# david-cortes/poismf

Measured on AMD Instinct MI355X. Metric: nonzeros/sec per full A+B sweep, higher is better.
Workload: dtype f32; 1 GPU; uniform 1000000x100000, 99949803 nnz (100000000 triplets, seed 1, duplicates summed), k=50, method=pg, maxupd=10, l2=1000, step=1e-09

## Files before the change

poismf_amd/csrc/poismf_hip.hip:

```cpp
#include <hip/hip_runtime.h>

#include <algorithm>
#include <atomic>
#include <cstdio>
#include <cstdlib>
#include <type_traits>

#include "plan.hpp"
#include "reg_eval.hpp"
#include "quad_eval.hpp"
#include "lane_eval.hpp"
#include "solvers.hpp"

#ifndef PMF_TU
#define PMF_TU -1
#endif
constexpr bool tu_has(int kmethod) { return PMF_TU == -1 || PMF_TU == kmethod; }

template <class EV, class = void> struct cold_constants : std::false_type {};
template <class EV> struct cold_constants<EV, std::void_t<decltype(EV::COLD_CONSTANTS)>> : std::integral_constant<bool, EV::COLD_CONSTANTS> {};

template <class EV, class = void> struct has_idle_tile : std::false_type {};
template <class EV> struct has_idle_tile<EV, std::void_t<decltype(&EV::idle_tile)>> : std::true_type {};

template <class EV, class T, int NC, int METHOD>
__device__ __forceinline__ void solve_row(const HalfArgs<T>& a, EV& ev, const T (&bs)[NC], unsigned lrow, unsigned nnz)
{
    const int k = a.geom.k;
    T* out = a.M + (size_t)(a.row_offset + lrow) * (size_t)k;
    T* out_p = a.Mp != nullptr ? a.Mp + (size_t)(a.row_offset + lrow) * (size_t)a.ldM : nullptr;
    T x[NC];
    if (nnz == 0) {
        T z = (T)0;
        asm volatile("" : "+v"(z));
        PMF_EW x[i] = z;
        ev.store_vec(out, x);
        if (out_p != nullptr) ev.store_vec(out_p, x);
        return;
    }
    ev.start_point(out, x);
    ev.n_eval = 0;

    T shift[NC];
    PMF_EW shift[i] = bs[i];
    const bool weighted = a.P.w != (T)1;
    if (weighted) {
        T cs[NC];
        PMF_EW cs[i] = (T)0;
        ev.tile_colsum(cs);
        T w_here = a.P.w;
        asm volatile("" : "+v"(w_here));
        const T wm1 = w_here - (T)1.;
        PMF_EW {
            shift[i] = cs[i] * wm1;
            shift[i] = shift[i] + bs[i];
        }
        if (METHOD == K_PG) {
            PMF_EW shift[i] = shift[i] * a.P.neg_step;
            if (a.P.neg_step2 != (T)1) { PMF_EW shift[i] = shift[i] * a.P.neg_step2; }
        }
    }

    SolveStats st;
    if constexpr (METHOD == K_EVAL) {
        T g[NC];
        double f;
        if (a.P.maxupd == 0) {
            f = (double)fun_single(ev, a.P, shift, x);
            grad_single(ev, a.P, shift, x, g, weighted);
        } else f = (double)fun_and_grad(ev, a.P, shift, x, g);
        ev.store_vec(out, g);
        if (out_p != nullptr) ev.store_vec(out_p, g);
        if (a.dec_rows != nullptr && ev.lane == 0 && ev.wid == 0 && ev.member == 0) {
            const unsigned long long fb = __builtin_bit_cast(unsigned long long, f);
            a.dec_rows[2 * (size_t)lrow] = (unsigned)fb;
            a.dec_rows[2 * (size_t)lrow + 1] = (unsigned)(fb >> 32);
        }
        return;
    } else if constexpr (METHOD == K_PG) {
        pg_row(ev, a.P, x, shift);
    } else if constexpr (METHOD == K_CG) {
        if constexpr (EV::MAY_CACHE) {
            if (a.P.limit_step && ev.pq_cap > 0 && nnz <= (unsigned)ev.pq_cap) cg_row_cached(ev, a.P, shift, x, weighted, st);
            else cg_row(ev, a.P, shift, x, weighted, st);
        } else cg_row(ev, a.P, shift, x, weighted, st);
    } else {
        T prev[NC];
        PMF_EW prev[i] = x[i];
        if (!a.reuse_prev) { PMF_EW x[i] = (T)1e-3; }
        (void)Tnc<T, NC, EV>::minimize(ev, a.P, shift, x, st);
        if (a.early_stop) {
            PMF_EW prev[i] = prev[i] - x[i];
            const T moved = ev.dot(prev, prev);
            if ((double)moved <= 1e-4 && ev.lane == 0 && ev.wid == 0 && ev.member == 0) atomicAdd(a.n_unchanged, 1u);
        }
    }
    ev.store_vec(out, x);
    if (out_p != nullptr) ev.store_vec(out_p, x);
#ifndef PMF_PROBE
    if (a.eval_rows != nullptr && ev.lane == 0 && ev.wid == 0 && ev.member == 0) a.eval_rows[lrow] += ev.n_eval;
#endif
    if (a.dec_rows != nullptr && ev.lane == 0 && ev.wid == 0 && ev.member == 0) {
        unsigned d0 = (unsigned)st.niter | ((unsigned)st.rc << 24), d1 = (unsigned)st.nfeval;
        if constexpr (cold_constants<EV>::value) asm volatile("" : "+v"(d0), "+v"(d1));
        a.dec_rows[2 * (size_t)lrow] = d0;
        a.dec_rows[2 * (size_t)lrow + 1] = d1;
    }
}

template <int METHOD, class T> __device__ __forceinline__ unsigned take_ticket(const HalfArgs<T>& a)
{
    unsigned st = 0u;
    if constexpr (METHOD != K_PG) {
        if (a.stop != nullptr) st = __hip_atomic_load(a.stop, __ATOMIC_RELAXED, __HIP_MEMORY_SCOPE_SYSTEM);
    }
    const unsigned t = atomicAdd(a.queue, 1u);
    return st != 0u ? 0xffffffffu : t;
}

template <class EV, class T, int NC, int METHOD, int NW>
__device__ __forceinline__ void sweep_rows(const HalfArgs<T>& a, EV& ev, unsigned char* smem)
{
    if (a.gate != nullptr && __hip_atomic_load(a.gate, __ATOMIC_RELAXED, __HIP_MEMORY_SCOPE_AGENT) == 0) return;
    ev.init(a.geom, a.F, smem);
    T bs[NC];
    ev.load_vec(a.bsum, bs);
    const RowDesc* desc = a.desc + a.perm_begin;
    if constexpr (EV::PIPELINED && (EV::PIPE_MW == 1 || (EV::PIPE_MW == 2 && METHOD == K_PG))) {
        unsigned r = blockIdx.x;
        auto ticket = [&]() -> unsigned {
            if (a.queue != nullptr) {
                if constexpr (NW > 1) {
                    unsigned* slot = ev.ticket_slot();
                    if (threadIdx.x == 0) *slot = take_ticket<METHOD>(a);
                    __syncthreads();
                    const unsigned t = uniform(*slot);
                    __syncthreads();
                    return t;
                }
                unsigned t = 0;
                if (ev.lane == 0) t = take_ticket<METHOD>(a);
                return uniform(t);
            }
            unsigned t = r;
            r += gridDim.x;
            if constexpr (METHOD != K_PG) {
                if (a.stop != nullptr && __hip_atomic_load(a.stop, __ATOMIC_RELAXED, __HIP_MEMORY_SCOPE_SYSTEM) != 0u) t = 0xffffffffu;
            }
            return t;
        };
        auto fetch = [&](unsigned t) -> RowDesc { return desc[t < a.nrows ? t : 0u]; };
        unsigned t0 = ticket(), t1 = ticket();
        RowDesc d0 = fetch(t0), d1 = fetch(t1);
        if (t0 < a.nrows) ev.fetch_meta(a.indices + (((unsigned long long)d0.p0_hi << 32) | d0.p0_lo), d0.nnz);
#ifdef PMF_PROBE
        unsigned probe_i = 0;
#endif
        while (t0 < a.nrows) {
            const unsigned long long p0 = ((unsigned long long)d0.p0_hi << 32) | d0.p0_lo;
            if (d0.nnz != 0) ev.gather(a.values + p0, d0.nnz);
            else if constexpr (has_idle_tile<EV>::value) ev.idle_tile();
            const unsigned t2 = ticket();
            const RowDesc d2 = fetch(t2);
            if (t1 < a.nrows) ev.fetch_meta(a.indices + (((unsigned long long)d1.p0_hi << 32) | d1.p0_lo), d1.nnz);
#ifdef PMF_PROBE
            ev.probe = (a.eval_rows != nullptr && blockIdx.x == 5 && threadIdx.x < WAVE && probe_i < 60) ? a.eval_rows + 16 * probe_i : nullptr;
            if (ev.probe != nullptr && ev.lane == 0) { ev.probe[10] = (unsigned)__builtin_amdgcn_s_memtime(); ev.probe[11] = d0.nnz; }
            probe_i++;
#endif
            solve_row<EV, T, NC, METHOD>(a, ev, bs, d0.lrow, d0.nnz);
            t0 = t1; d0 = d1;
            t1 = t2; d1 = d2;
        }
        return;
    } else {
        unsigned r = blockIdx.x;
        for (;;) {
            if (a.queue != nullptr) {
                if constexpr (NW > 1) {
                    unsigned* next_row = ev.ticket_slot();
                    if (threadIdx.x == 0) *next_row = take_ticket<METHOD>(a);
                    __syncthreads();
                    r = uniform(*next_row);
                    __syncthreads();
                } else {
                    unsigned t = 0;
                    if (ev.lane == 0) t = take_ticket<METHOD>(a);
                    r = uniform(t);
                }
            }
            if (r >= a.nrows) break;
            if constexpr (METHOD != K_PG) {
                if (a.queue == nullptr && a.stop != nullptr && uniform(__hip_atomic_load(a.stop, __ATOMIC_RELAXED, __HIP_MEMORY_SCOPE_SYSTEM)) != 0u) break;
            }
            const RowDesc d = desc[r];
            r += gridDim.x;
            const unsigned nnz = uniform(d.nnz);
            const unsigned long long p0 = ((unsigned long long)uniform(d.p0_hi) << 32) | uniform(d.p0_lo);
            if (nnz != 0) ev.begin_row(a.indices + p0, a.values + p0, nnz);
            solve_row<EV, T, NC, METHOD>(a, ev, bs, uniform(d.lrow), nnz);
        }
    }
}

template <class T, int NC, int METHOD, int SL, int NW>
__global__ __launch_bounds__(WAVE* NW) void half_sweep_kernel(const HalfArgs<T> a)
{
    extern __shared__ __attribute__((aligned(16))) unsigned char smem[];
    constexpr bool PF = SL > 0 && METHOD != K_TNCG;
    RowEval<T, NC, SL, NW, PF> ev;
    if constexpr (NW > 1) {
        if (a.arrive != nullptr && threadIdx.x == 0) atomicAdd(a.arrive, 1u);
    }
#ifdef PMF_TIMING
    const unsigned long long t_kernel = __builtin_amdgcn_s_memtime();
#endif
    sweep_rows<RowEval<T, NC, SL, NW, PF>, T, NC, METHOD, NW>(a, ev, smem);
#ifdef PMF_TIMING
    ev.tacc[5] = __builtin_amdgcn_s_memtime() - t_kernel;
    if (ev.lane == 0 && ev.wid == 0)
        for (int q = 0; q < 6; q++) atomicAdd(&g_pmf_timing[q], ev.tacc[q]);
#endif
}

template <class EV, class T, int NC, int METHOD>
__device__ __forceinline__ void team_rows(const HalfArgs<T>& a, EV& ev, unsigned char* smem)
{
    if (a.arrive != nullptr && threadIdx.x == 0) atomicAdd(a.arrive, 1u);
    ev.init(a.geom, a.F, smem);
    T bs[NC];
    ev.load_vec(a.bsum, bs);
    const RowDesc* desc = a.desc + a.perm_begin;
    const unsigned M = a.team_members;
    unsigned* box = ev.ticket_slot();
    if (threadIdx.x == 0) {
        const unsigned n = atomicAdd((unsigned*)a.team_buf, 1u);
        box[0] = n / M;
        box[1] = n % M;
    }
    __syncthreads();
    const unsigned team = uniform(box[0]);
    ev.member = (int)uniform(box[1]);
    __syncthreads();
    if ((size_t)(team + 1) * gt_team_words(M) + GT_HEAD_WORDS > GT_BUF_BYTES / 8) return;
    ev.tm_M = (int)M;
    ev.tm_seq = 0;
    ev.tm_words = a.team_buf + GT_HEAD_WORDS + (size_t)team * gt_team_words(M);
    ev.tm_err = a.team_err;
    ev.tm_spin = a.team_spin;
    unsigned long long* mail = ev.tm_words;
    constexpr unsigned END = 0xffffffffu;
    if (threadIdx.x == 0) atomicAdd((unsigned*)(mail + 2), 1u);
    if (a.team_spin <= 1u && threadIdx.x == 0) __hip_atomic_store(a.team_err, 1u, __ATOMIC_RELAXED, __HIP_MEMORY_SCOPE_AGENT);
    if (ev.wid == 0) {
        for (unsigned spins = 0;; spins++) {
            if (a.team_spin <= 1u) break;
            if (uniform((unsigned)gt_load(mail + 2)) >= M) break;
            if ((spins & 255u) == 255u) {
                if (uniform(__hip_atomic_load(a.team_err, __ATOMIC_RELAXED, __HIP_MEMORY_SCOPE_AGENT)) != 0) break;
                if (uniform(__hip_atomic_load(a.queue, __ATOMIC_RELAXED, __HIP_MEMORY_SCOPE_AGENT)) >= a.nrows) break;
            }
            if ((spins >> 6) > a.team_spin) { __hip_atomic_store(a.team_err, 1u, __ATOMIC_RELAXED, __HIP_MEMORY_SCOPE_AGENT); break; }
            __builtin_amdgcn_s_sleep(8);
        }
    }
    __syncthreads();
    for (unsigned rowno = 1;; rowno++) {
        if (ev.wid == 0) {
            unsigned tk = END;
            if (ev.member == 0) {
                unsigned t0 = 0;
                if (ev.lane == 0) t0 = take_ticket<METHOD>(a);
                tk = uniform(t0);
                if (tk >= a.nrows || uniform(__hip_atomic_load(a.team_err, __ATOMIC_RELAXED, __HIP_MEMORY_SCOPE_AGENT)) != 0) tk = END;
                gt_store(mail + (rowno & 1u), ((unsigned long long)rowno << 32) | tk);
            } else {
                unsigned seen = uniform(__hip_atomic_load(a.queue, __ATOMIC_RELAXED, __HIP_MEMORY_SCOPE_AGENT));
                for (unsigned spins = 0;; spins++) {
                    const unsigned long long v = gt_load(mail + (rowno & 1u));
                    const unsigned hi = uniform((unsigned)(v >> 32)), lo = uniform((unsigned)v);
                    if (hi == rowno) { tk = lo; break; }
                    if ((spins & 255u) == 255u) {
                        if (uniform(__hip_atomic_load(a.team_err, __ATOMIC_RELAXED, __HIP_MEMORY_SCOPE_AGENT)) != 0) break;
                        const unsigned q = uniform(__hip_atomic_load(a.queue, __ATOMIC_RELAXED, __HIP_MEMORY_SCOPE_AGENT));
                        if (q != seen) { seen = q; spins = 0; }
                        else if (rowno == 1u && q >= a.nrows) break;
                    }
                    if (spins > a.team_spin) { __hip_atomic_store(a.team_err, 1u, __ATOMIC_RELAXED, __HIP_MEMORY_SCOPE_AGENT); break; }
                    __builtin_amdgcn_s_sleep(4);
                }
            }
            box[0] = tk;
        }
        __syncthreads();
        const unsigned t = uniform(box[0]);
        __syncthreads();
        if (t >= a.nrows) break;
        const RowDesc d = desc[t];
        const unsigned nnz = uniform(d.nnz);
        const unsigned long long p0 = ((unsigned long long)uniform(d.p0_hi) << 32) | uniform(d.p0_lo);
        const unsigned S = ((nnz + M - 1u) / M + (EV::TEAM_ROUND - 1u)) / EV::TEAM_ROUND * EV::TEAM_ROUND;
        const unsigned off = (unsigned)ev.member * S;
        const unsigned mine = off < nnz ? (nnz - off < S ? nnz - off : S) : 0u;
        ev.begin_row(a.indices + p0 + (mine ? off : 0u), a.values + p0 + (mine ? off : 0u), mine);
        solve_row<EV, T, NC, METHOD>(a, ev, bs, uniform(d.lrow), nnz);
    }
}
template <class T, int NC, int METHOD, int SL, int NW>
__global__ __launch_bounds__(WAVE* NW) void half_sweep_giant_kernel(const HalfArgs<T> a)
{
    extern __shared__ __attribute__((aligned(16))) unsigned char smem[];
    constexpr bool PF = SL > 0 && METHOD != K_TNCG;
    using EV = RowEval<T, NC, SL, NW, PF, true>;
    EV ev;
    team_rows<EV, T, NC, METHOD>(a, ev, smem);
}
template <class T, int METHOD, int KS, int LV, int LA, int LL, int NW, int LP>
__global__ __launch_bounds__(WAVE* NW) __attribute__((amdgpu_waves_per_eu(1, 1))) void half_sweep_lane_team_kernel(const HalfArgs<T> a)
{
    using EV = LaneEval<T, KS, LV, LA, LL, NW, false, LP, 0, true>;
    __shared__ __attribute__((aligned(16))) unsigned char smem[EV::SMEM_BYTES];
    EV ev;
    team_rows<EV, T, EV::NC, METHOD>(a, ev, smem);
}

#ifndef PMF_PG_EXTRA
#define PMF_PG_EXTRA 56
#endif
#ifndef PMF_CG_EXTRA
#define PMF_CG_EXTRA 120
#endif
#ifndef PMF_TNC_EXTRA
#define PMF_TNC_EXTRA 100
#endif
constexpr int reg_waves(int tile_regs, int method)
{
    const int need = tile_regs + (method == K_PG ? PMF_PG_EXTRA : method == K_CG ? PMF_CG_EXTRA : PMF_TNC_EXTRA);
    for (int w : { 8, 6, 5, 4, 3, 2 })
        if ((512 / w) / 8 * 8 >= need) return w;
    return 1;
}
template <class T, int METHOD, int G, int NS> constexpr bool reg_pairs() { return METHOD == K_PG && sizeof(T) == 4 && G == 16 && NS == 1; }
template <class T, int METHOD, int S, int G, int NS>
__global__ __launch_bounds__(WAVE) __attribute__((amdgpu_waves_per_eu(reg_waves(4 * S * NS, METHOD)))) void half_sweep_reg_kernel(const HalfArgs<T> a)
{
    using EV = RegEval<T, S, G, NS, 1, 1, reg_pairs<T, METHOD, G, NS>()>;
    EV ev;
    constexpr int SMEM = EV::SMEM_BYTES;
    __shared__ __attribute__((aligned(16))) unsigned char smem[SMEM > 0 && METHOD == K_CG ? SMEM : 16];
#ifdef PMF_TIMING
    const unsigned long long t_kernel = __builtin_amdgcn_s_memtime();
#endif
    sweep_rows<EV, T, EV::NC, METHOD, 1>(a, ev, smem);
#ifdef PMF_TIMING
    if (ev.lane == 0) atomicAdd(&g_pmf_timing[5], __builtin_amdgcn_s_memtime() - t_kernel);
#endif
}

template <int Q>
__global__ __launch_bounds__(WAVE) __attribute__((amdgpu_waves_per_eu(reg_waves(14 * Q, K_PG)))) void half_sweep_quad_kernel(const HalfArgs<float> a)
{
    using EV = QuadEval<Q>;
    EV ev;
    sweep_rows<EV, float, EV::NC, K_PG, 1>(a, ev, nullptr);
}

constexpr int regw_waves(int tile_regs, int method, int nw)
{
    const int w = reg_waves(tile_regs + (method == K_PG ? 8 : 0), method);
    return nw >= 16 && w < 4 ? 4 : (nw >= 8 && w < 2 ? 2 : w);
}
template <class T, int METHOD, int S, int G, int NS, int NW>
__global__ __launch_bounds__(WAVE* NW) __attribute__((amdgpu_waves_per_eu(regw_waves(4 * S * NS, METHOD, NW)))) void half_sweep_regw_kernel(const HalfArgs<T> a)
{
    using EV = RegEval<T, S, G, NS, NW>;
    __shared__ __attribute__((aligned(16))) unsigned char smem[EV::SMEM_BYTES];
    EV ev;
    sweep_rows<EV, T, EV::NC, METHOD, NW>(a, ev, smem);
}

template <class T, int METHOD, int S, int G, int NS, int NW, int M>
__global__ __launch_bounds__(WAVE* NW) __attribute__((amdgpu_waves_per_eu(1))) void half_sweep_team_kernel(const HalfArgs<T> a)
{
    using EV = RegEval<T, S, G, NS, NW, M>;
    constexpr int NC = EV::NC;
    __shared__ __attribute__((aligned(16))) unsigned char smem[EV::SMEM_BYTES];
    EV ev;
    ev.init(a.geom, a.F, smem);
    T bs[NC];
    ev.load_vec(a.bsum, bs);
    const RowDesc* desc = a.desc + a.perm_begin;
    unsigned* arrive = (unsigned*)a.team_buf;
    unsigned* err = a.team_err;
    unsigned* box = ev.ticket_slot();
    if (threadIdx.x == 0) {
        unsigned xcc = 0;
        if (gridDim.x >= 8u * 4u * (unsigned)M) {
            asm volatile("s_getreg_b32 %0, hwreg(HW_REG_XCC_ID)" : "=s"(xcc));
            xcc &= 7u;
        }
        const unsigned n = atomicAdd(arrive + xcc, 1u);
        box[0] = xcc * TEAM_SLOTS_PER_XCD + n / (unsigned)M;
        box[1] = n % (unsigned)M;
        if (n / (unsigned)M >= TEAM_SLOTS_PER_XCD) __hip_atomic_store(err, 2u, __ATOMIC_RELAXED, __HIP_MEMORY_SCOPE_AGENT);
    }
    __syncthreads();
    const unsigned team = uniform(box[0]) % TEAM_SLOTS;
    ev.member = (int)uniform(box[1]);
    __syncthreads();
    ev.team_words = a.team_buf + TEAM_HEAD_WORDS + (size_t)team * TEAM_WORDS;
    ev.team_err = err;
    ev.team_spin = a.team_spin;
    unsigned long long* mail = ev.team_words;
    unsigned long long* here = ev.team_words + 2;
    constexpr unsigned END = 0xffffffffu;
    if (ev.member != 0 && threadIdx.x == 0) gran_store(here + ev.member, 1ull);

    if (ev.member == 0) {
        if (threadIdx.x == 0) {
            unsigned full = 0;
            unsigned seen = __hip_atomic_load(a.queue, __ATOMIC_RELAXED, __HIP_MEMORY_SCOPE_AGENT);
            for (unsigned spins = 0; !full; spins++) {
                full = 1;
                for (int m = 1; m < M; m++) full &= gran_load(here + m) != 0ull;
                if (full) break;
                const unsigned q = __hip_atomic_load(a.queue, __ATOMIC_RELAXED, __HIP_MEMORY_SCOPE_AGENT);
                if (q >= a.nrows || __hip_atomic_load(err, __ATOMIC_RELAXED, __HIP_MEMORY_SCOPE_AGENT) != 0) break;
                if (q != seen) { seen = q; spins = 0; }
                if (spins > a.team_spin) { __hip_atomic_store(err, 3u, __ATOMIC_RELAXED, __HIP_MEMORY_SCOPE_AGENT); break; }
                __builtin_amdgcn_s_sleep(8);
            }
            box[0] = full;
        }
        __syncthreads();
        const bool full = uniform(box[0]) != 0;
        __syncthreads();
        if (!full) {
            if (threadIdx.x == 0) gran_store(mail + 1, ((unsigned long long)1u << 32) | END);
            return;
        }
    }

    auto next_ticket = [&](unsigned rowno_next) -> unsigned {
        if (ev.member == 0) {
            if (threadIdx.x == 0) {
                box[0] = take_ticket<METHOD>(a);
                gran_store(mail + (rowno_next & 1u), ((unsigned long long)rowno_next << 32) | (box[0] < a.nrows ? box[0] : END));
            }
        } else if (threadIdx.x == 0) {
            unsigned long long v = 0;
            unsigned seen = __hip_atomic_load(a.queue, __ATOMIC_RELAXED, __HIP_MEMORY_SCOPE_AGENT);
            for (unsigned spins = 0;; spins++) {
                v = gran_load(mail + (rowno_next & 1u));
                if ((unsigned)(v >> 32) == rowno_next) break;
                if ((spins & 255u) == 255u) {
                    if (__hip_atomic_load(err, __ATOMIC_RELAXED, __HIP_MEMORY_SCOPE_AGENT) != 0) { v = END; break; }
                    const unsigned q = __hip_atomic_load(a.queue, __ATOMIC_RELAXED, __HIP_MEMORY_SCOPE_AGENT);
                    if (rowno_next == 1u && q != seen) { seen = q; spins = 0; }
                }
                if (spins > a.team_spin) {
                    __hip_atomic_store(err, 1u, __ATOMIC_RELAXED, __HIP_MEMORY_SCOPE_AGENT);
                    v = END;
                    break;
                }
                __builtin_amdgcn_s_sleep(2);
            }
            box[0] = (unsigned)v;
        }
        __syncthreads();
        const unsigned tk = uniform(box[0]);
        __syncthreads();
        return tk;
    };
    auto row_of = [&](unsigned tk, unsigned& nnz, unsigned long long& p0, unsigned& lrow) {
        const RowDesc d = desc[tk < a.nrows ? tk : 0u];
        nnz = uniform(d.nnz);
        p0 = ((unsigned long long)uniform(d.p0_hi) << 32) | uniform(d.p0_lo);
        lrow = uniform(d.lrow);
    };
    unsigned rowno = 1;
    unsigned t = next_ticket(1);
    unsigned nnz = 0, lrow = 0;
    unsigned long long p0 = 0;
    row_of(t, nnz, p0, lrow);
    if (t < a.nrows) ev.fetch_meta(a.indices + p0, nnz);
    while (t < a.nrows) {
        if (__hip_atomic_load(err, __ATOMIC_RELAXED, __HIP_MEMORY_SCOPE_AGENT) != 0) break;
#ifdef PMF_PROBE
        const unsigned long long t_row0 = __builtin_amdgcn_s_memtime();
        ev.probe_wait = 0;
#endif
        ev.gather(a.values + p0, nnz);
        const unsigned t_next = next_ticket(rowno + 1);
        unsigned nnz_next = 0, lrow_next = 0;
        unsigned long long p0_next = 0;
        row_of(t_next, nnz_next, p0_next, lrow_next);
        if (t_next < a.nrows) ev.fetch_meta(a.indices + p0_next, nnz_next);
#ifdef PMF_PROBE
        {
            T probe_sum[NC];
            PMF_EW probe_sum[i] = (T)0;
            ev.tile_touch(probe_sum);
            ev.probe_acc[4] += __builtin_amdgcn_s_memtime() - t_row0;
            if (probe_sum[0] == (T)123.456) ev.probe_acc[6]++;
        }
#endif
        solve_row<EV, T, NC, METHOD>(a, ev, bs, lrow, nnz);
#ifdef PMF_PROBE
        if (a.eval_rows != nullptr && threadIdx.x == 0 && ev.member == 0)
            a.eval_rows[lrow] = (unsigned)std::min<unsigned long long>(0xffffu, ev.probe_wait >> 8) |
                                ((unsigned)std::min<unsigned long long>(0xffffu, (__builtin_amdgcn_s_memtime() - t_row0) >> 8) << 16);
        ev.probe_acc[5] += __builtin_amdgcn_s_memtime() - t_row0;
        ev.probe_acc[6] += ev.probe_wait;
#endif
        rowno++;
        t = t_next; nnz = nnz_next; p0 = p0_next; lrow = lrow_next;
    }
#ifdef PMF_PROBE
    if (threadIdx.x == 0 && ev.member == 0)
        for (int q = 0; q < 8; q++) atomicAdd(a.team_buf + 8 + q, ev.probe_acc[q]);
#endif
}

template <bool SMALL> constexpr bool lane_two() { return SMALL; }
template <class T, int METHOD, int KS, int LV, int LA, int LL, int NW, bool SMALL, int LP = 0, int TX = 0, int KU = 0>
__global__ __launch_bounds__(WAVE* NW) __attribute__((amdgpu_waves_per_eu(lane_two<SMALL>() ? 2 : 1, lane_two<SMALL>() ? 2 : 1))) void half_sweep_lane_kernel(const HalfArgs<T> a)
{
    using EV = LaneEval<T, KS, LV, LA, LL, NW, SMALL, LP, TX, false, KU>;
    __shared__ __attribute__((aligned(16))) unsigned char smem[EV::SMEM_BYTES];
    EV ev;
    sweep_rows<EV, T, EV::NC, METHOD, NW>(a, ev, smem);
}

namespace {

using std::integral_constant;
constexpr int MAX_DEVICES = 64;

template <auto Kern, int THREADS> int launch_grid(const OneLaunch& o, const HalfArgs<real_t>& a, unsigned grid, size_t lds = 0)
{
    if (o.dry) return 0;
    hipLaunchKernelGGL(Kern, dim3(grid), dim3(THREADS), lds, o.stream, a);
    HIP_TRY(hipGetLastError());
    return 0;
}
template <auto Kern, int THREADS> int launch_occ(const OneLaunch& o, const HalfArgs<real_t>& a)
{
    if (o.dry) return 0;
    static std::atomic<int> occ_cache{0};
    int occ = occ_cache.load(std::memory_order_relaxed);
    if (occ == 0) {
        int n = 0;
        HIP_TRY(hipOccupancyMaxActiveBlocksPerMultiprocessor(&n, reinterpret_cast<const void*>(Kern), THREADS, 0));
        occ = std::max(1, n);
        occ_cache.store(occ, std::memory_order_relaxed);
    }
    return launch_grid<Kern, THREADS>(o, a, (unsigned)std::min<size_t>(a.nrows, (size_t)o.num_cu * (size_t)occ * o.grid_mult));
}
template <auto Kern, int THREADS> int launch_lds(const OneLaunch& o, const HalfArgs<real_t>& a)
{
    if (o.dry) return 0;
    static std::atomic<bool> attr_set[MAX_DEVICES];
    const int dev = o.device >= 0 && o.device < MAX_DEVICES ? o.device : 0;
    if (!attr_set[dev].load(std::memory_order_acquire) || dev != o.device) {
        HIP_TRY(hipFuncSetAttribute(reinterpret_cast<const void*>(Kern), hipFuncAttributeMaxDynamicSharedMemorySize, (int)LDS_PER_CU));
        attr_set[dev].store(true, std::memory_order_release);
    }
    return launch_grid<Kern, THREADS>(o, a, o.grid, o.lds);
}

template <class F> int with_method(int method, F f)
{
    switch (method) {
        case POISMF_PG:
            if constexpr (tu_has(K_PG)) return f(integral_constant<int, K_PG>{});
            else return 1;
        case POISMF_CG:
            if constexpr (tu_has(K_CG)) return f(integral_constant<int, K_CG>{});
            else return 1;
        case POISMF_EVAL:
            if constexpr (tu_has(K_EVAL)) return f(integral_constant<int, K_EVAL>{});
            else return 1;
        default:
            if constexpr (tu_has(K_TNCG)) return f(integral_constant<int, K_TNCG>{});
            else return 1;
    }
}
template <class F> int with_steps(int S, F f)
{
    switch (S) {
#define X(NZ) case (NZ) / REG_JG: return f(integral_constant<int, (NZ) / REG_JG>{});
        PMF_REG_SIZES(X)
#undef X
    }
    return 1;
}
template <class F> int with_slots(const OneLaunch& o, F f)
{
    if (o.s_load == SPECIAL_SL_A) return f(integral_constant<int, SLOT_ELEMS>{}, integral_constant<int, SPECIAL_SL_A>{});
    if (o.s_load == SPECIAL_SL_B) return f(integral_constant<int, SLOT_ELEMS>{}, integral_constant<int, SPECIAL_SL_B>{});
    switch (o.spl) {
        case 1: return f(integral_constant<int, 1 * SLOT_ELEMS>{}, integral_constant<int, 0>{});
        case 2: return f(integral_constant<int, 2 * SLOT_ELEMS>{}, integral_constant<int, 0>{});
    }
    return 1;
}

template <int NW> int launch_bin(int method, const OneLaunch& o, const HalfArgs<real_t>& a)
{
    return with_slots(o, [&](auto nc, auto sl) {
        return with_method(method, [&](auto m) {
            return launch_lds<half_sweep_kernel<real_t, decltype(nc)::value, decltype(m)::value, decltype(sl)::value, NW>, WAVE * NW>(o, a);
        });
    });
}
int launch_giant(int method, const OneLaunch& o, const HalfArgs<real_t>& a)
{
    return with_slots(o, [&](auto nc, auto sl) {
        if constexpr (tu_has(K_TNCG)) {
            if (method == POISMF_TNCG)
                return launch_lds<half_sweep_giant_kernel<real_t, decltype(nc)::value, K_TNCG, decltype(sl)::value, LONG_NW>, WAVE * LONG_NW>(o, a);
        }
        return 1;
    });
}

int launch_reg(int method, const OneLaunch& o, const HalfArgs<real_t>& a)
{
    return with_method(method, [&](auto m) {
        return with_steps(o.reg_S, [&](auto s) {
            constexpr int M = decltype(m)::value, S = decltype(s)::value;
            const int ns = REG_NS_MAX == 1 || o.s_load <= REG_G ? 1 : 2;
            if constexpr (reg_instance(M, S, 1)) {
                if (ns == 1) return launch_occ<half_sweep_reg_kernel<real_t, M, S, REG_G, 1>, WAVE>(o, a);
            }
            if constexpr (reg_instance(M, S, 2)) {
                if (ns == 2) return launch_occ<half_sweep_reg_kernel<real_t, M, S, REG_G, 2>, WAVE>(o, a);
            }
            return 1;
        });
    });
}
int launch_quad(int method, const OneLaunch& o, const HalfArgs<real_t>& a)
{
    if (method != POISMF_PG || a.geom.k != QUAD_K || a.geom.ldF != QUAD_LD) return 1;
    return with_steps(o.reg_S, [&](auto s) {
        if constexpr (tu_has(K_PG) && sizeof(real_t) == 4 && PMF_REG_QUAD != 0 && REG_G == 16)
            return launch_occ<half_sweep_quad_kernel<decltype(s)::value * REG_JG / 16>, WAVE>(o, a);
        else return 1;
    });
}
template <int NW> int launch_regw(int method, const OneLaunch& o, const HalfArgs<real_t>& a)
{
    return with_method(method, [&](auto m) {
        return with_steps(o.reg_S, [&](auto s) {
            constexpr int M = decltype(m)::value, S = decltype(s)::value;
            if constexpr (regw_instance(M, S, NW)) {
                if (REG_G == 16 || o.s_load <= REG_G) return launch_occ<half_sweep_regw_kernel<real_t, M, S, REG_G, 1, NW>, WAVE * NW>(o, a);
                if constexpr (REG_G != 16) return launch_occ<half_sweep_regw_kernel<real_t, M, S, REG_G, 2, NW>, WAVE * NW>(o, a);
            }
            return 1;
        });
    });
}
template <int M, int S> int launch_team(int method, const OneLaunch& o, const HalfArgs<real_t>& a)
{
    if constexpr ((tu_has(K_CG) || tu_has(K_EVAL)) && sizeof(real_t) == 8 && REG_G == 16) {
        constexpr int KM = tu_has(K_CG) ? K_CG : K_EVAL;
        if (method != (KM == K_CG ? POISMF_CG : POISMF_EVAL)) return 1;
        const unsigned grid = (unsigned)std::min<size_t>((size_t)a.nrows * M, (size_t)o.num_cu / M * M);
        return launch_grid<half_sweep_team_kernel<real_t, KM, S, REG_G, 2, TEAM_NW, M>, WAVE * TEAM_NW>(o, a, grid);
    } else return 1;
}

template <int METHOD, int KS, int LV, int LA, int LL, int NW, bool SMALL, int LP, int TX, int KU> int launch_lane(const OneLaunch& o, const HalfArgs<real_t>& a)
{
    using EV = LaneEval<real_t, KS, LV, LA, LL, NW, SMALL, LP, TX, false, KU>;
    const int occ = std::max(1, std::min((lane_two<SMALL>() ? 8 : 4) / NW, (int)(LDS_PER_CU / (size_t)EV::SMEM_BYTES)));
    const unsigned grid = (unsigned)std::min<size_t>(a.nrows, (size_t)o.num_cu * (size_t)occ * o.grid_mult);
    return launch_grid<half_sweep_lane_kernel<real_t, METHOD, KS, LV, LA, LL, NW, SMALL, LP, TX, KU>, WAVE * NW>(o, a, grid);
}
int launch_lane_shape(int method, const OneLaunch& o, const HalfArgs<real_t>& a)
{
    return with_method(method, [&](auto m) {
        constexpr int M = decltype(m)::value;
#define X(FOR, KS, LV, LA, LL, NW, SMALL, LP, TX, KU)                                                  \
        if constexpr ((((FOR) >> M) & 1u) != 0 && ((KU) == 0 || PMF_LANE_KU50 != 0)) {                 \
            if (o.s_load == (KS) && o.lane == LaneShape{ LV, LA, LL, NW, SMALL, LP, TX, KU })          \
                return launch_lane<M, KS, LV, LA, LL, NW, (SMALL) != 0, LP, TX, KU>(o, a);             \
        }
        PMF_LANE_INSTANCES(X)
#undef X
        return 1;
    });
}
int launch_lane_team(int method, const OneLaunch& o, const HalfArgs<real_t>& a)
{
    return with_method(method, [&](auto m) {
        if constexpr (decltype(m)::value == K_TNCG && sizeof(real_t) == 8) {
            if (o.s_load == LANE_TEAM_KS && o.lane == LANE_TEAM_SHAPE)
                return launch_grid<half_sweep_lane_team_kernel<real_t, K_TNCG, LANE_TEAM_KS, LANE_TEAM_SHAPE.lv, LANE_TEAM_SHAPE.la, LANE_TEAM_SHAPE.ll, LANE_TEAM_SHAPE.waves,
                                                               LANE_TEAM_SHAPE.lp>, WAVE * LANE_TEAM_SHAPE.waves>(o, a, o.grid);
        }
        return 1;
    });
}

int launch_one_here(int method, const OneLaunch& o, const HalfArgs<real_t>& a)
{
    switch (o.engine) {
        case Engine::LaneTeam: return launch_lane_team(method, o, a);
        case Engine::Lane: return launch_lane_shape(method, o, a);
#ifndef PMF_LANE_ONLY
        case Engine::RegTeam:
#define X(M, S) if (o.team == (M) && o.reg_S == (S)) return launch_team<M, S>(method, o, a);
            PMF_TEAM_SHAPES(X)
#undef X
            return 1;
        case Engine::Reg: return o.quad != 0 ? launch_quad(method, o, a) : launch_reg(method, o, a);
        case Engine::RegW:
            switch (o.nw) {
                case 2: return launch_regw<2>(method, o, a);
                case 4: return launch_regw<4>(method, o, a);
                case 8: return launch_regw<8>(method, o, a);
            }
            return 1;
        case Engine::Giant: return launch_giant(method, o, a);
        case Engine::LdsLong: return launch_bin<LONG_NW>(method, o, a);
        case Engine::Lds: return launch_bin<1>(method, o, a);
#else
        default: return 1;
#endif
    }
    return 1;
}
}

#if PMF_TU == 1 || PMF_TU == -1
int pmf_launch_one_tu1(int method, const OneLaunch& o, const HalfArgs<real_t>& a) { return launch_one_here(method, o, a); }
#endif
#if PMF_TU == 2 || PMF_TU == -1
int pmf_launch_one_tu2(int method, const OneLaunch& o, const HalfArgs<real_t>& a) { return launch_one_here(method, o, a); }
#endif
#if PMF_TU == 3 || PMF_TU == -1
int pmf_launch_one_tu3(int method, const OneLaunch& o, const HalfArgs<real_t>& a) { return launch_one_here(method, o, a); }
#endif
#if PMF_TU == 4 || PMF_TU == -1
int pmf_launch_one_tu4(int method, const OneLaunch& o, const HalfArgs<real_t>& a) { return launch_one_here(method, o, a); }
#endif

#ifdef PMF_TIMING
int pmf_read_timing(unsigned long long* out)
{
    (void)hipDeviceSynchronize();
    if (hipMemcpyFromSymbol(out, HIP_SYMBOL(g_pmf_timing), sizeof(unsigned long long) * 8) != hipSuccess) return 1;
    unsigned long long z[8] = {0, 0, 0, 0, 0, 0, 0, 0};
    return hipMemcpyToSymbol(HIP_SYMBOL(g_pmf_timing), z, sizeof(z)) != hipSuccess;
}
#endif
```

poismf_amd/csrc/quad_eval.hpp:

```cpp
#pragma once
#include "reg_eval.hpp"

namespace pmf {

#define PMF_QFOLD4(Q, A, B) \
    "v_add_f32_dpp " Q ", " A ", " A " row_shl:4 row_mask:0xf bank_mask:0x5\n\t" \
    "v_add_f32_dpp " Q ", " B ", " B " row_shr:4 row_mask:0xf bank_mask:0xa\n\t"
__device__ __forceinline__ void quad_fold14(const float (&p)[14], float (&q)[7])
{
    asm("s_nop 1\n\t"
        PMF_QFOLD4("%0", "%7", "%14")
        PMF_QFOLD4("%1", "%8", "%15")
        PMF_QFOLD4("%2", "%9", "%16")
        PMF_QFOLD4("%3", "%10", "%17")
        PMF_QFOLD4("%4", "%11", "%18")
        PMF_QFOLD4("%5", "%12", "%19")
        PMF_QFOLD4("%6", "%13", "%20")
        : "=&v"(q[0]), "=&v"(q[1]), "=&v"(q[2]), "=&v"(q[3]), "=&v"(q[4]), "=&v"(q[5]), "=&v"(q[6])
        : "v"(p[0]), "v"(p[1]), "v"(p[2]), "v"(p[3]), "v"(p[4]), "v"(p[5]), "v"(p[6]),
          "v"(p[7]), "v"(p[8]), "v"(p[9]), "v"(p[10]), "v"(p[11]), "v"(p[12]), "v"(p[13]));
}
__device__ __forceinline__ void quad_fold7(const float (&q)[7], float (&r)[4])
{
    asm("s_nop 1\n\t"
        PMF_FOLD2("row_ror:8", "0x3", "0xc", "%0", "%4", "%8")
        PMF_FOLD2("row_ror:8", "0x3", "0xc", "%1", "%5", "%9")
        PMF_FOLD2("row_ror:8", "0x3", "0xc", "%2", "%6", "%10")
        PMF_FOLD1("row_ror:8", "%3", "%7")
        : "=&v"(r[0]), "=&v"(r[1]), "=&v"(r[2]), "=&v"(r[3])
        : "v"(q[0]), "v"(q[1]), "v"(q[2]), "v"(q[3]), "v"(q[4]), "v"(q[5]), "v"(q[6]));
}

template <int Q> struct QuadEval {
    using T = float;
    static_assert(Q >= 1 && Q <= 10, "one to ten steps of sixteen nonzeros");
    typedef float V2 __attribute__((ext_vector_type(2)));
    struct __attribute__((packed, aligned(4))) U4 { float v[4]; };
    struct __attribute__((packed, aligned(4))) U2 { float v[2]; };
    static constexpr int K = 50;
    static constexpr int NP = 7;
    static constexpr int NE = 2 * NP;
    static constexpr int NC = 1;
    static constexpr int NB = (Q + 3) / 4;
    static constexpr int NW = 1, M = 1;
    static constexpr bool PIPELINED = true;
    static constexpr int PIPE_MW = 1;
    static constexpr bool FUSED_SUMS = false, PREFETCH = false, MAY_CACHE = false, CACHED_GRAD = false;
    static constexpr bool PG_LEAN = true;
    static constexpr int SMEM_BYTES = 0;

    V2 t[Q][NP];
    V2 a[NP];
    T xr[NB];
    unsigned idx_n[NB];
    const T* F;
    unsigned zero_row;
    int k, ldF;
    int lane, q, wid, member;
    int jlane;
    int dim;
    bool primary;
    bool cls1, cls2, cls16, cls32;
    int xor32_addr;
    int quad_addr;
    unsigned nnz;
    unsigned n_eval;
#ifdef PMF_PROBE
    unsigned* probe = nullptr;
#endif

    static __host__ __device__ constexpr int acc_of(int quad)
    {
        const int n = ((quad >> 3) & 1) + 2 * ((quad >> 2) & 1) + 4 * ((quad >> 1) & 1);
        return (n == 7 ? 3 : n) + 7 * (quad & 1);
    }
    static __host__ __device__ constexpr int quad_of(int e)
    {
        const int n = e % 7;
        return (e / 7) + 2 * ((n >> 2) & 1) + 4 * ((n >> 1) & 1) + 8 * (n & 1);
    }
    static __host__ __device__ constexpr int dim_of(int q_, int e) { return e < 12 ? 12 * q_ + e : (q_ == 0 ? 48 + (e - 12) : -1); }

    __device__ __forceinline__ void init(const TileGeom& geo, const T* F_, unsigned char*)
    {
        lane = lane_id();
        F = F_;
        k = geo.k; ldF = geo.ldF; zero_row = geo.zero_row;
        q = lane & 3; wid = 0; member = 0;
        jlane = 16 * q + (lane >> 2);
        cls1 = (lane & 1) != 0; cls2 = (lane & 2) != 0; cls16 = (lane & 16) != 0; cls32 = (lane & 32) != 0;
        const int quad = lane >> 2;
        const int e = acc_of(quad);
        dim = e < 12 ? 12 * q + e : (q == 0 ? 48 + (e - 12) : -1);
        primary = dim >= 0 && (quad >> 1) != 7;
        xor32_addr = (lane ^ 32) << 2;
        quad_addr = q << 2;
        asm volatile("" : "+v"(xor32_addr), "+v"(quad_addr));
    }

    __device__ __forceinline__ void load_vec(const T* p, T (&x)[NC]) const { x[0] = dim >= 0 ? p[dim >= 0 ? dim : 0] : (T)0; }
    __device__ __forceinline__ void start_point(const T* mrow, T (&x)[NC]) const { load_vec(mrow, x); }
    __device__ __forceinline__ void store_vec(T* p, const T (&x)[NC]) const
    {
        if (primary) p[dim] = x[0];
    }

    __device__ __forceinline__ void fetch_meta(const unsigned* ind, unsigned nnz_row)
    {
#pragma unroll
        for (int b = 0; b < NB; b++) {
            const unsigned j = (unsigned)(64 * b + jlane);
            idx_n[b] = j < nnz_row ? ind[j] : zero_row;
        }
    }
    __device__ __forceinline__ void begin_row(const unsigned* ind, const T* val, unsigned nnz_row)
    {
        fetch_meta(ind, nnz_row);
        gather(val, nnz_row);
    }
    __device__ __forceinline__ unsigned* ticket_slot() const { return nullptr; }
    __device__ __forceinline__ void gather(const T* val, unsigned nnz_row)
    {
        nnz = nnz_row;
        unsigned idx[NB];
#pragma unroll
        for (int b = 0; b < NB; b++) {
            const unsigned j = (unsigned)(64 * b + jlane);
            idx[b] = idx_n[b];
            xr[b] = j < nnz ? val[j] : (T)0;
        }
        const unsigned rowbytes = (unsigned)ldF * (unsigned)sizeof(T);
        const unsigned main_off = (unsigned)q * 48u;
        const unsigned tail_mul = q == 0 ? rowbytes : 0u;
        const unsigned tail_off = q == 0 ? 192u : __umul24(zero_row, rowbytes);
        static_for<0, Q>([&](auto sc) {
            constexpr int s = decltype(sc)::value;
            const unsigned c = group_bcast<4, s % 4>(idx[s / 4]);
            const char* base = (const char*)F + (size_t)(__umul24(c, rowbytes) + main_off);
            const U4 v0 = *(const U4*)base;
            const U4 v1 = *(const U4*)(base + 16);
            const U4 v2 = *(const U4*)(base + 32);
            const U2 w = *(const U2*)((const char*)F + (size_t)(__umul24(c, tail_mul) + tail_off));
            t[s][0] = (V2){ v0.v[0], v0.v[1] }; t[s][1] = (V2){ v0.v[2], v0.v[3] };
            t[s][2] = (V2){ v1.v[0], v1.v[1] }; t[s][3] = (V2){ v1.v[2], v1.v[3] };
            t[s][4] = (V2){ v2.v[0], v2.v[1] }; t[s][5] = (V2){ v2.v[2], v2.v[3] };
            t[s][6] = (V2){ w.v[0], w.v[1] };
        });
    }
    __device__ __forceinline__ void idle_tile()
    {
        asm volatile("" ::: "memory");
#pragma unroll
        for (int s = 0; s < Q; s++) {
#pragma unroll
            for (int e = 0; e < NP; e++) t[s][e] = (V2){ (T)0, (T)0 };
        }
    }

    __device__ __forceinline__ void set_point_as_is(const T (&x)[NC])
    {
#define PMF_QPERM(D, E) "ds_bpermute_b32 " D ", %14, %15 offset:%" E "\n\t"
        float r[NE];
        asm volatile(PMF_QPERM("%0", "16") PMF_QPERM("%1", "17") PMF_QPERM("%2", "18") PMF_QPERM("%3", "19") PMF_QPERM("%4", "20")
                     PMF_QPERM("%5", "21") PMF_QPERM("%6", "22") PMF_QPERM("%7", "23") PMF_QPERM("%8", "24") PMF_QPERM("%9", "25")
                     PMF_QPERM("%10", "26") PMF_QPERM("%11", "27") PMF_QPERM("%12", "28") PMF_QPERM("%13", "29")
                     "s_waitcnt lgkmcnt(0)"
                     : "=&v"(r[0]), "=&v"(r[1]), "=&v"(r[2]), "=&v"(r[3]), "=&v"(r[4]), "=&v"(r[5]), "=&v"(r[6]), "=&v"(r[7]), "=&v"(r[8]), "=&v"(r[9]),
                       "=&v"(r[10]), "=&v"(r[11]), "=&v"(r[12]), "=&v"(r[13])
                     : "v"(quad_addr), "v"(x[0]), "n"(16 * quad_of(0)), "n"(16 * quad_of(1)), "n"(16 * quad_of(2)), "n"(16 * quad_of(3)),
                       "n"(16 * quad_of(4)), "n"(16 * quad_of(5)), "n"(16 * quad_of(6)), "n"(16 * quad_of(7)), "n"(16 * quad_of(8)), "n"(16 * quad_of(9)),
                       "n"(16 * quad_of(10)), "n"(16 * quad_of(11)), "n"(16 * quad_of(12)), "n"(16 * quad_of(13)));
#undef PMF_QPERM
#pragma unroll
        for (int e = 0; e < NP; e++) a[e] = (V2){ r[2 * e], r[2 * e + 1] };
    }
    __device__ __forceinline__ void set_point(const T (&x)[NC]) { set_point_as_is(x); }

    template <int N> __device__ __forceinline__ T quad_transpose_sum(const T (&p)[4]) const
    {
        T r0, r1;
        if constexpr (N >= 2) r0 = fold_pair<0xB1>(cls1, p[0], p[1]);
        else r0 = fold_one<0xB1>(p[0]);
        if constexpr (N == 4) r1 = fold_pair<0xB1>(cls1, p[2], p[3]);
        else if constexpr (N == 3) r1 = fold_one<0xB1>(p[2]);
        if constexpr (N >= 3) return fold_pair<0x4E>(cls2, r0, r1);
        else return fold_one<0x4E>(r0);
    }

    __device__ __forceinline__ T cross_quads(const T (&part)[NE]) const
    {
        T l4[7], l8[4];
        quad_fold14(part, l4);
        quad_fold7(l4, l8);
        T l16[2];
#pragma unroll
        for (int i = 0; i < 2; i++) {
            const T own = cls16 ? l8[i + 2] : l8[i];
            const T send = cls16 ? l8[i] : l8[i + 2];
            l16[i] = own + __builtin_bit_cast(T, __builtin_amdgcn_ds_swizzle(__builtin_bit_cast(int, send), 0x401f));
        }
        const T own = cls32 ? l16[1] : l16[0];
        const T send = cls32 ? l16[0] : l16[1];
        return own + __builtin_bit_cast(T, __builtin_amdgcn_ds_bpermute(xor32_addr, __builtin_bit_cast(int, send)));
    }

    template <bool WANT_F, bool WANT_G, bool FROM_CACHE = false, bool FRESH = false> __device__ __forceinline__ double eval(T sgn, T (&acc)[NC], T* = nullptr)
    {
        static_assert(!WANT_F && WANT_G && !FROM_CACHE, "the quad engine evaluates PG's gradient only");
        n_eval++;
        PMF_STAMP(*this, 0);
        V2 part2[NP];
        static_for<0, NB>([&](auto bc) {
            constexpr int b = decltype(bc)::value;
            constexpr int n = (Q - 4 * b) < 4 ? (Q - 4 * b) : 4;
            T p[4];
            V2 s2[n];
#pragma unroll
            for (int u = 0; u < n; u++) s2[u] = t[4 * b + u][0] * a[0];
#pragma unroll
            for (int e = 1; e < NP; e++) {
#pragma unroll
                for (int u = 0; u < n; u++) s2[u] = __builtin_elementwise_fma(t[4 * b + u][e], a[e], s2[u]);
            }
#pragma unroll
            for (int u = 0; u < 4; u++) p[u] = u < n ? s2[u < n ? u : 0].x + s2[u < n ? u : 0].y : (T)0;
            const T pred = quad_transpose_sum<n>(p);
            const bool on = (unsigned)(64 * b + jlane) < nnz;
            const T coef = on ? coef_div(sgn * xr[b], pred) : (T)0;
            static_for<0, n>([&](auto uc) {
                constexpr int u = decltype(uc)::value;
                const T c = group_bcast<4, u>(coef);
                const V2 c2 = { c, c };
#pragma unroll
                for (int e = 0; e < NP; e++) {
                    if constexpr (b == 0 && u == 0) part2[e] = c2 * t[0][e];
                    else part2[e] = __builtin_elementwise_fma(c2, t[4 * b + u][e], part2[e]);
                }
            });
        });
        PMF_STAMP(*this, 5);
        T part[NE];
#pragma unroll
        for (int e = 0; e < NP; e++) { part[2 * e] = part2[e].x; part[2 * e + 1] = part2[e].y; }
        const T g = cross_quads(part);
        acc[0] = FRESH ? g : acc[0] + g;
        PMF_STAMP(*this, 6);
        return 0.0;
    }

    __device__ __forceinline__ void tile_colsum(T (&acc)[NC])
    {
        T part[NE];
#pragma unroll
        for (int i = 0; i < NE; i++) part[i] = (T)0;
#pragma unroll
        for (int s = 0; s < Q; s++) {
#pragma unroll
            for (int e = 0; e < NP; e++) { part[2 * e] += t[s][e].x; part[2 * e + 1] += t[s][e].y; }
        }
        acc[0] += cross_quads(part);
    }
};

}
```

Baseline: 12.10 billion nnz/s.

## Distribute k=50 tail dims across quad lanes instead of replicating per step

Each quad previously held a 7th V2 slot per step for the two tail dimensions of K=50. Only q==0 loaded real data into it and the other lanes held zeros. Now the tail pair for step s is loaded only by lane q==s%4 into a per-batch tt register, and its contribution is added directly to the prediction and the gradient partials. A DPP quad reduction folds the tail sum at the end. This cuts tile registers from 14*Q to 12*Q+2*NB and drops the zero-row tail loads, which should allow more waves per EU. The cost is extra FMAs per batch and an extra DPP reduction, plus a change to the lane-to-dimension mapping.

```diff
diff --git a/poismf_amd/csrc/poismf_hip.hip b/poismf_amd/csrc/poismf_hip.hip
--- a/poismf_amd/csrc/poismf_hip.hip
+++ b/poismf_amd/csrc/poismf_hip.hip
@@ -358,7 +358,7 @@
 }
 
 template <int Q>
-__global__ __launch_bounds__(WAVE) __attribute__((amdgpu_waves_per_eu(reg_waves(14 * Q, K_PG)))) void half_sweep_quad_kernel(const HalfArgs<float> a)
+__global__ __launch_bounds__(WAVE) __attribute__((amdgpu_waves_per_eu(reg_waves(QuadEval<Q>::TILE_REGS, K_PG)))) void half_sweep_quad_kernel(const HalfArgs<float> a)
 {
     using EV = QuadEval<Q>;
     EV ev;
diff --git a/poismf_amd/csrc/quad_eval.hpp b/poismf_amd/csrc/quad_eval.hpp
--- a/poismf_amd/csrc/quad_eval.hpp
+++ b/poismf_amd/csrc/quad_eval.hpp
@@ -30,6 +30,15 @@
         : "=&v"(r[0]), "=&v"(r[1]), "=&v"(r[2]), "=&v"(r[3])
         : "v"(q[0]), "v"(q[1]), "v"(q[2]), "v"(q[3]), "v"(q[4]), "v"(q[5]), "v"(q[6]));
 }
+__device__ __forceinline__ float quad_tail_sum(float g)
+{
+    asm("s_nop 1\n\t"
+        "v_add_f32_dpp %0, %0, %0 quad_perm:[1,0,3,2] row_mask:0x6 bank_mask:0x8\n\t"
+        "s_nop 1\n\t"
+        "v_add_f32_dpp %0, %0, %0 quad_perm:[2,3,0,1] row_mask:0x6 bank_mask:0x8"
+        : "+v"(g));
+    return g;
+}
 
 template <int Q> struct QuadEval {
     using T = float;
@@ -38,19 +47,23 @@
     struct __attribute__((packed, aligned(4))) U4 { float v[4]; };
     struct __attribute__((packed, aligned(4))) U2 { float v[2]; };
     static constexpr int K = 50;
-    static constexpr int NP = 7;
-    static constexpr int NE = 2 * NP;
+    static constexpr int NP = 6;
+    static constexpr int NA = NP + 1;
+    static constexpr int NE = 2 * NA;
     static constexpr int NC = 1;
     static constexpr int NB = (Q + 3) / 4;
+    static constexpr int TILE_REGS = 2 * NP * Q + 2 * NB;
     static constexpr int NW = 1, M = 1;
     static constexpr bool PIPELINED = true;
     static constexpr int PIPE_MW = 1;
     static constexpr bool FUSED_SUMS = false, PREFETCH = false, MAY_CACHE = false, CACHED_GRAD = false;
     static constexpr bool PG_LEAN = true;
     static constexpr int SMEM_BYTES = 0;
+    static_assert(K == 4 * 2 * NP + 2, "four lanes of twelve elements and a tail of two");
 
     V2 t[Q][NP];
-    V2 a[NP];
+    V2 tt[NB];
+    V2 a[NA];
     T xr[NB];
     unsigned idx_n[NB];
     const T* F;
@@ -79,7 +92,7 @@
         const int n = e % 7;
         return (e / 7) + 2 * ((n >> 2) & 1) + 4 * ((n >> 1) & 1) + 8 * (n & 1);
     }
-    static __host__ __device__ constexpr int dim_of(int q_, int e) { return e < 12 ? 12 * q_ + e : (q_ == 0 ? 48 + (e - 12) : -1); }
+    static __host__ __device__ constexpr int dim_of(int q_, int e) { return e < 2 * NP ? 2 * NP * q_ + e : 8 * NP + (e - 2 * NP); }
 
     __device__ __forceinline__ void init(const TileGeom& geo, const T* F_, unsigned char*)
     {
@@ -91,14 +104,14 @@
         cls1 = (lane & 1) != 0; cls2 = (lane & 2) != 0; cls16 = (lane & 16) != 0; cls32 = (lane & 32) != 0;
         const int quad = lane >> 2;
         const int e = acc_of(quad);
-        dim = e < 12 ? 12 * q + e : (q == 0 ? 48 + (e - 12) : -1);
-        primary = dim >= 0 && (quad >> 1) != 7;
+        dim = dim_of(q, e);
+        primary = (quad >> 1) != 7 && (e < 2 * NP || q == 0);
         xor32_addr = (lane ^ 32) << 2;
         quad_addr = q << 2;
         asm volatile("" : "+v"(xor32_addr), "+v"(quad_addr));
     }
 
-    __device__ __forceinline__ void load_vec(const T* p, T (&x)[NC]) const { x[0] = dim >= 0 ? p[dim >= 0 ? dim : 0] : (T)0; }
+    __device__ __forceinline__ void load_vec(const T* p, T (&x)[NC]) const { x[0] = p[dim]; }
     __device__ __forceinline__ void start_point(const T* mrow, T (&x)[NC]) const { load_vec(mrow, x); }
     __device__ __forceinline__ void store_vec(T* p, const T (&x)[NC]) const
     {
@@ -131,8 +144,8 @@
         }
         const unsigned rowbytes = (unsigned)ldF * (unsigned)sizeof(T);
         const unsigned main_off = (unsigned)q * 48u;
-        const unsigned tail_mul = q == 0 ? rowbytes : 0u;
-        const unsigned tail_off = q == 0 ? 192u : __umul24(zero_row, rowbytes);
+#pragma unroll
+        for (int b = 0; b < NB; b++) tt[b] = (V2){ (T)0, (T)0 };
         static_for<0, Q>([&](auto sc) {
             constexpr int s = decltype(sc)::value;
             const unsigned c = group_bcast<4, s % 4>(idx[s / 4]);
@@ -140,11 +153,13 @@
             const U4 v0 = *(const U4*)base;
             const U4 v1 = *(const U4*)(base + 16);
             const U4 v2 = *(const U4*)(base + 32);
-            const U2 w = *(const U2*)((const char*)F + (size_t)(__umul24(c, tail_mul) + tail_off));
             t[s][0] = (V2){ v0.v[0], v0.v[1] }; t[s][1] = (V2){ v0.v[2], v0.v[3] };
             t[s][2] = (V2){ v1.v[0], v1.v[1] }; t[s][3] = (V2){ v1.v[2], v1.v[3] };
             t[s][4] = (V2){ v2.v[0], v2.v[1] }; t[s][5] = (V2){ v2.v[2], v2.v[3] };
-            t[s][6] = (V2){ w.v[0], w.v[1] };
+            if (q == s % 4) {
+                const U2 w = *(const U2*)((const char*)F + (size_t)(__umul24(idx[s / 4], rowbytes) + 192u));
+                tt[s / 4] = (V2){ w.v[0], w.v[1] };
+            }
         });
     }
     __device__ __forceinline__ void idle_tile()
@@ -155,6 +170,8 @@
 #pragma unroll
             for (int e = 0; e < NP; e++) t[s][e] = (V2){ (T)0, (T)0 };
         }
+#pragma unroll
+        for (int b = 0; b < NB; b++) tt[b] = (V2){ (T)0, (T)0 };
     }
 
     __device__ __forceinline__ void set_point_as_is(const T (&x)[NC])
@@ -172,7 +189,7 @@
                        "n"(16 * quad_of(10)), "n"(16 * quad_of(11)), "n"(16 * quad_of(12)), "n"(16 * quad_of(13)));
 #undef PMF_QPERM
 #pragma unroll
-        for (int e = 0; e < NP; e++) a[e] = (V2){ r[2 * e], r[2 * e + 1] };
+        for (int e = 0; e < NA; e++) a[e] = (V2){ r[2 * e], r[2 * e + 1] };
     }
     __device__ __forceinline__ void set_point(const T (&x)[NC]) { set_point_as_is(x); }
 
@@ -201,7 +218,8 @@
         }
         const T own = cls32 ? l16[1] : l16[0];
         const T send = cls32 ? l16[0] : l16[1];
-        return own + __builtin_bit_cast(T, __builtin_amdgcn_ds_bpermute(xor32_addr, __builtin_bit_cast(int, send)));
+        static_assert(quad_of(2 * NP) == 11 && quad_of(2 * NP + 1) == 7, "quad_tail_sum's masks: DPP rows 2 and 1, bank 3");
+        return quad_tail_sum(own + __builtin_bit_cast(T, __builtin_amdgcn_ds_bpermute(xor32_addr, __builtin_bit_cast(int, send))));
     }
 
     template <bool WANT_F, bool WANT_G, bool FROM_CACHE = false, bool FRESH = false> __device__ __forceinline__ double eval(T sgn, T (&acc)[NC], T* = nullptr)
@@ -209,7 +227,7 @@
         static_assert(!WANT_F && WANT_G && !FROM_CACHE, "the quad engine evaluates PG's gradient only");
         n_eval++;
         PMF_STAMP(*this, 0);
-        V2 part2[NP];
+        V2 part2[NA];
         static_for<0, NB>([&](auto bc) {
             constexpr int b = decltype(bc)::value;
             constexpr int n = (Q - 4 * b) < 4 ? (Q - 4 * b) : 4;
@@ -224,9 +242,15 @@
             }
 #pragma unroll
             for (int u = 0; u < 4; u++) p[u] = u < n ? s2[u < n ? u : 0].x + s2[u < n ? u : 0].y : (T)0;
-            const T pred = quad_transpose_sum<n>(p);
+            T pred = quad_transpose_sum<n>(p);
+            pred = __builtin_fmaf(tt[b].x, a[NP].x, __builtin_fmaf(tt[b].y, a[NP].y, pred));
             const bool on = (unsigned)(64 * b + jlane) < nnz;
             const T coef = on ? coef_div(sgn * xr[b], pred) : (T)0;
+            {
+                const V2 c2 = { coef, coef };
+                if constexpr (b == 0) part2[NP] = c2 * tt[0];
+                else part2[NP] = __builtin_elementwise_fma(c2, tt[b], part2[NP]);
+            }
             static_for<0, n>([&](auto uc) {
                 constexpr int u = decltype(uc)::value;
                 const T c = group_bcast<4, u>(coef);
@@ -241,7 +265,7 @@
         PMF_STAMP(*this, 5);
         T part[NE];
 #pragma unroll
-        for (int e = 0; e < NP; e++) { part[2 * e] = part2[e].x; part[2 * e + 1] = part2[e].y; }
+        for (int e = 0; e < NA; e++) { part[2 * e] = part2[e].x; part[2 * e + 1] = part2[e].y; }
         const T g = cross_quads(part);
         acc[0] = FRESH ? g : acc[0] + g;
         PMF_STAMP(*this, 6);
@@ -258,6 +282,8 @@
 #pragma unroll
             for (int e = 0; e < NP; e++) { part[2 * e] += t[s][e].x; part[2 * e + 1] += t[s][e].y; }
         }
+#pragma unroll
+        for (int b = 0; b < NB; b++) { part[2 * NP] += tt[b].x; part[2 * NP + 1] += tt[b].y; }
         acc[0] += cross_quads(part);
     }
 };
```

New measurement: 12.33 billion nnz/s, median of 6. 1.02x the previous value.
